# StefanSko/mcmc-db

Measured on AMD Instinct MI355X. Metric: validated param-draws/sec, higher is better.
Workload: dtype f64; 1 GPU; single posteriordb-shaped model, 4x10000x100 synthetic draws per GPU (BASELINE config 1; AR(1) chains, ties and a shifted chain; SURVEY 8(d) C1); layout=pcn, statistics=mean,std,q5,q50,q95,split_rhat,ess_bulk,ess_tail

## Files before the change

mcmc-db_amd/csrc/mcr_device.hpp:

```cpp
#pragma once
#include <hip/hip_runtime.h>
#include <stdint.h>

namespace mcr {

using i64 = long long;
using u32 = unsigned int;
using u64 = unsigned long long;

constexpr int kWave = 64;

template <int CTRL>
__device__ __forceinline__ double dpp_f64(double v)
{
    const int lo = __builtin_amdgcn_mov_dpp(__double2loint(v), CTRL, 0xf, 0xf, true);
    const int hi = __builtin_amdgcn_mov_dpp(__double2hiint(v), CTRL, 0xf, 0xf, true);
    return __hiloint2double(hi, lo);
}
__device__ __forceinline__ double readlane_f64(double v, int lane)
{
    return __hiloint2double(__builtin_amdgcn_readlane(__double2hiint(v), lane),
                            __builtin_amdgcn_readlane(__double2loint(v), lane));
}
constexpr int kDppXor1 = 0xB1, kDppXor2 = 0x4E, kDppRor4 = 0x124, kDppRor8 = 0x128;

__device__ __forceinline__ double row_sum(double v)
{
    v += dpp_f64<kDppXor1>(v); v += dpp_f64<kDppXor2>(v); v += dpp_f64<kDppRor4>(v); v += dpp_f64<kDppRor8>(v);
    return v;
}
template <int CTRL>
__device__ __forceinline__ u32 dpp_u32(u32 v) { return (u32)__builtin_amdgcn_mov_dpp((int)v, CTRL, 0xf, 0xf, true); }
__device__ __forceinline__ u32 row_min_u32(u32 v)
{
    v = min(v, dpp_u32<kDppXor1>(v)); v = min(v, dpp_u32<kDppXor2>(v));
    v = min(v, dpp_u32<kDppRor4>(v)); v = min(v, dpp_u32<kDppRor8>(v));
    return v;
}
__device__ __forceinline__ u32 row_max_u32(u32 v)
{
    v = max(v, dpp_u32<kDppXor1>(v)); v = max(v, dpp_u32<kDppXor2>(v));
    v = max(v, dpp_u32<kDppRor4>(v)); v = max(v, dpp_u32<kDppRor8>(v));
    return v;
}
__device__ __forceinline__ double wave_sum(double v)
{
    v = row_sum(v);
    return (readlane_f64(v, 0) + readlane_f64(v, 16)) + (readlane_f64(v, 32) + readlane_f64(v, 48));
}
template <int CTRL, int ROW_MASK>
__device__ __forceinline__ double dpp_f64_or_zero(double v)
{
    const int lo = __builtin_amdgcn_update_dpp(0, __double2loint(v), CTRL, ROW_MASK, 0xf, false);
    const int hi = __builtin_amdgcn_update_dpp(0, __double2hiint(v), CTRL, ROW_MASK, 0xf, false);
    return __hiloint2double(hi, lo);
}
__device__ __forceinline__ double wave_excl_scan(double v, double& total)
{
    double incl = v;
    incl += dpp_f64_or_zero<0x111, 0xf>(incl);
    incl += dpp_f64_or_zero<0x112, 0xf>(incl);
    incl += dpp_f64_or_zero<0x114, 0xf>(incl);
    incl += dpp_f64_or_zero<0x118, 0xf>(incl);
    incl += dpp_f64_or_zero<0x142, 0xa>(incl);
    incl += dpp_f64_or_zero<0x143, 0xc>(incl);
    total = readlane_f64(incl, 63);
    return incl - v;
}

__device__ __forceinline__ int row_lane(int v, int j)
{
#define MCR_RL(J) case J: return __builtin_amdgcn_update_dpp(0, v, 0x150 + J, 0xf, 0xf, false);
    switch (j & 15) {
        MCR_RL(0) MCR_RL(1) MCR_RL(2) MCR_RL(3) MCR_RL(4) MCR_RL(5) MCR_RL(6) MCR_RL(7)
        MCR_RL(8) MCR_RL(9) MCR_RL(10) MCR_RL(11) MCR_RL(12) MCR_RL(13) MCR_RL(14)
        default: return __builtin_amdgcn_update_dpp(0, v, 0x15F, 0xf, 0xf, false);
    }
#undef MCR_RL
}

template <int CTRL, int ROW_MASK, int OLD>
__device__ __forceinline__ int dpp_i32_or(int v) { return __builtin_amdgcn_update_dpp(OLD, v, CTRL, ROW_MASK, 0xf, false); }

__device__ __forceinline__ u32 wave_excl_scan_u32(u32 v, u32& total)
{
    int incl = (int)v;
    incl += dpp_i32_or<0x111, 0xf, 0>(incl); incl += dpp_i32_or<0x112, 0xf, 0>(incl);
    incl += dpp_i32_or<0x114, 0xf, 0>(incl); incl += dpp_i32_or<0x118, 0xf, 0>(incl);
    incl += dpp_i32_or<0x142, 0xa, 0>(incl);
    incl += dpp_i32_or<0x143, 0xc, 0>(incl);
    total = (u32)__builtin_amdgcn_readlane(incl, 63);
    return (u32)incl - v;
}

__device__ __forceinline__ int wave_prefix_max(int v, int& excl)
{
    v = max(v, dpp_i32_or<0x111, 0xf, -1>(v)); v = max(v, dpp_i32_or<0x112, 0xf, -1>(v));
    v = max(v, dpp_i32_or<0x114, 0xf, -1>(v)); v = max(v, dpp_i32_or<0x118, 0xf, -1>(v));
    v = max(v, dpp_i32_or<0x142, 0xa, -1>(v)); v = max(v, dpp_i32_or<0x143, 0xc, -1>(v));
    excl = dpp_i32_or<0x138, 0xf, -1>(v);
    return v;
}
__device__ __forceinline__ int wave_suffix_min(int v, int& excl)
{
    constexpr int kMax = 0x7fffffff;
    v = min(v, dpp_i32_or<0x101, 0xf, kMax>(v)); v = min(v, dpp_i32_or<0x102, 0xf, kMax>(v));
    v = min(v, dpp_i32_or<0x104, 0xf, kMax>(v)); v = min(v, dpp_i32_or<0x108, 0xf, kMax>(v));
    const int r1 = __builtin_amdgcn_readlane(v, 16), r2 = __builtin_amdgcn_readlane(v, 32), r3 = __builtin_amdgcn_readlane(v, 48);
    const int row = (threadIdx.x & 63) >> 4;
    const int m23 = min(r2, r3), m123 = min(r1, m23);
    const int above = (row == 0) ? m123 : ((row == 1) ? m23 : ((row == 2) ? r3 : kMax));
    v = min(v, above);
    excl = dpp_i32_or<0x130, 0xf, kMax>(v);
    return v;
}

template <int NT>
__device__ __forceinline__ double block_sum(double v, double* red)
{
    v = wave_sum(v);
    __syncthreads();
    if ((threadIdx.x & 63) == 0) red[threadIdx.x >> 6] = v;
    __syncthreads();
    double r = 0.0;
#pragma unroll
    for (int w = 0; w < NT / kWave; ++w) r += red[w];
    return r;
// ... 143 lines not shown
```

mcmc-db_amd/csrc/mcr_diag.hpp:

```cpp
#pragma once
#include "mcr_device.hpp"

namespace mcr {

constexpr int kSeg = 2048;
#ifndef MCR_LAG1
#define MCR_LAG1 64
#endif
constexpr int kLag1 = MCR_LAG1;
constexpr int kSegRec = kLag1 + 12;
constexpr int kMoreBlocks = 3;
constexpr int kLag2 = kLag1 + 64 * kMoreBlocks;
constexpr int kLongGroup = 256;
constexpr int kLongSlots = 2;
enum SegField { SG_S = kLag1, SG_S0, SG_Q0, SG_S1, SG_Q1, SG_MIN, SG_MAX, SG_MIN0, SG_MAX0, SG_MIN1, SG_MAX1 };

__device__ __forceinline__ i64 pos8(i64 j) { return j + ((j >> 3) << 1); }

__device__ __forceinline__ double zdec(const double* __restrict__ ztab, u32 code, i64 M)
{
    const u32 cmax = (u32)(2 * M - 1);
    return ztab[code < cmax ? code : cmax];
}

// ... 39 lines not shown
    }
    __syncthreads();
    if (ph == 0) {
#pragma unroll
        for (int li = 0; li < LPL; ++li) wred[w * 64 + g * LPL + li] = acc[li];
    }
    __syncthreads();
    if (tid < LPL * LG) {
        double t = 0.0;
#pragma unroll
        for (int ww = 0; ww < NW; ++ww) t += wred[ww * 64 + tid];
        tot[tid] = t;
    }
    __syncthreads();
}

template <int NT, int LG = 8>
__device__ __forceinline__ void seg_reduce_rows(double (&acc)[8], double* tot, double* scr)
{
    constexpr int NW = NT / kWave;
    static_assert(LG == 8 || LG == 4, "8 or 4 lag groups of 8 lags");
    const int tid = threadIdx.x, lane = tid & 63, w = tid >> 6;
    const int g = lane & (LG - 1), row = lane >> 4;
#pragma unroll
    for (int li = 0; li < 8; ++li) {
        if (LG == 4) acc[li] += dpp_f64<kDppRor4>(acc[li]);
        acc[li] += dpp_f64<kDppRor8>(acc[li]);
    }
    __syncthreads();
    if ((lane & 15) < LG) {
#pragma unroll
        for (int li = 0; li < 8; ++li) scr[(w * 4 + row) * 64 + g * 8 + li] = acc[li];
    }
    __syncthreads();
    if (tid < LG * 8) {
        double t = 0.0;
#pragma unroll
        for (int r = 0; r < NW * 4; ++r) t += scr[r * 64 + tid];
        tot[tid] = t;
    }
    __syncthreads();
}

template <int NT, int SEG, bool FIRST>
__global__ __launch_bounds__(NT) void k_acov_seg(const u32* __restrict__ zb, const u32* __restrict__ zt,
                                                 const double* __restrict__ ztab, i64 M,
                                                 const i64* __restrict__ off, int C, i64 n, i64 nh, int nseg,
                                                 const unsigned* __restrict__ more, double* __restrict__ rec, int kind_sel)
{
    constexpr int NW = NT / kWave;
    static_assert(SEG % 128 == 0, "spans of the widest tile are 128 draws");
    static_assert(kLag1 == 64 || kLag1 == 32, "tier 1 is one or half a lag block");
    constexpr int WIN = FIRST ? SEG + 80 : SEG + 64 * kMoreBlocks + 80;
    constexpr int LX = WIN / 8 * 10;
    constexpr int NLD = (WIN + NT - 1) / NT;
    static_assert(LX >= NW * 4 * 64, "the reduction scratch aliases the staged window");
    __shared__ __attribute__((aligned(16))) double sx[LX];
    __shared__ __attribute__((aligned(16))) double scr2[FIRST ? 8 : NW * 4 * 64];
    __shared__ double tot[64];
    __shared__ double wred[NW * 4 * 8];

    const int tid = threadIdx.x;
    const int seg = blockIdx.x, c = blockIdx.y;
    const i64 pk = (kind_sel < 0) ? (i64)blockIdx.z : 2 * (i64)blockIdx.z + kind_sel, p = pk >> 1;
    const int kind = (int)(pk & 1);
    if (!FIRST && more[pk] == 0u) return;
    const u32* zc = (kind ? zt : zb) + p * M + off[c];
    const i64 nc = off[c + 1] - off[c], hc = nc / 2;
    const i64 hspan = (hc > 0) ? hc + nh : 0;
    const i64 nload = (n > hspan) ? n : hspan;
    const i64 s0 = (i64)seg * SEG;
    const int seglen = (int)((n - s0 < 0) ? 0 : ((n - s0 < (i64)SEG) ? n - s0 : (i64)SEG));

    if (FIRST) {
        auto rel = [&](i64 x) -> int { const i64 d = x - s0; return (int)(d < 0 ? 0 : (d > WIN ? WIN : d)); };
        const int r_load = rel(nload);
        const int r_n = rel(n);
        const int own = (r_load < SEG) ? r_load : SEG;
        const int own_n = (own < r_n) ? own : r_n;
        auto clip = [&](int x) -> int { return x < own ? x : own; };
        const int a0 = (hc > 0) ? clip(rel(0)) : 0, a1 = (hc > 0) ? clip(rel(nh)) : 0;
        const int b0 = (hc > 0) ? clip(rel(hc)) : 0, b1 = (hc > 0) ? clip(rel(hc + nh)) : 0;
        double S = 0.0, S0 = 0.0, Q0 = 0.0, S1 = 0.0, Q1 = 0.0;
        u32 cmin = 0xFFFFFFFFu, cmax = 0u;
        u32 c0min = 0xFFFFFFFFu, c0max = 0u, c1min = 0xFFFFFFFFu, c1max = 0u;
        double v[NLD];
        u32 cd[NLD];
#pragma unroll
        for (int u = 0; u < NLD; ++u) {
            const int j = u * NT + tid;
            cd[u] = (j < r_load) ? zc[s0 + j] : 0u;
            v[u] = (j < r_load) ? zdec(ztab, cd[u], M) : 0.0;
        }
        const int jw0 = __builtin_amdgcn_readfirstlane(tid & ~63);
#define MCR_IN_WINDOW(lo, hi, BODY)                                                        \
        if (jw >= (lo) && jw + 64 <= (hi)) { BODY }                                        \
        else if (jw + 64 > (lo) && jw < (hi)) { if (j >= (lo) && j < (hi)) { BODY } }
#pragma unroll
        for (int u = 0; u < NLD; ++u) {
            const int jw = u * NT + jw0, j = u * NT + tid;
            const double x = v[u];
            MCR_IN_WINDOW(0, own_n, S += x; cmin = min(cmin, cd[u]); cmax = max(cmax, cd[u]);)
            MCR_IN_WINDOW(a0, a1, S0 += x; Q0 = fma(x, x, Q0); c0min = min(c0min, cd[u]); c0max = max(c0max, cd[u]);)
            MCR_IN_WINDOW(b0, b1, S1 += x; Q1 = fma(x, x, Q1); c1min = min(c1min, cd[u]); c1max = max(c1max, cd[u]);)
            if (j < WIN) sx[pos8(j)] = (j < r_n) ? x : 0.0;
        }
#undef MCR_IN_WINDOW
        S = row_sum(S); S0 = row_sum(S0); Q0 = row_sum(Q0); S1 = row_sum(S1); Q1 = row_sum(Q1);
        cmin = row_min_u32(cmin); cmax = row_max_u32(cmax);
        c0min = row_min_u32(c0min); c0max = row_max_u32(c0max); c1min = row_min_u32(c1min); c1max = row_max_u32(c1max);
        static_assert(NW * 4 * 4 <= 64, "the four half-window fields of every DPP row fit `tot`");
        if ((tid & 15) == 0) {
            double* q = wred + (tid >> 4) * 8;
            q[0] = S; q[1] = S0; q[2] = Q0; q[3] = S1; q[4] = Q1; q[5] = (double)cmin; q[6] = (double)cmax;
            double* q2 = tot + (tid >> 4) * 4;
            q2[0] = (double)c0min; q2[1] = (double)c0max; q2[2] = (double)c1min; q2[3] = (double)c1max;
        }
        __syncthreads();
        double* r = rec + ((pk * C + c) * (i64)nseg + seg) * kSegRec;
        if (tid < 11) {
            const double* src = (tid < 7) ? wred + tid : tot + (tid - 7);
            const int stride = (tid < 7) ? 8 : 4;
            double t = src[0];
            for (int w = 1; w < NW * 4; ++w) {
                const double x = src[w * stride];
                t = (tid < 5) ? t + x : (((tid & 1) == 1) ? fmin(t, x) : fmax(t, x));
            }
            r[SG_S + tid] = t;
        }
        double acc[8];
#pragma unroll
        for (int i = 0; i < 8; ++i) acc[i] = 0.0;
        seg_accumulate<NT, kLag1 / 8, 8>(sx, sx, seglen, acc);
        seg_reduce_rows<NT, kLag1 / 8>(acc, tot, sx);
        if (tid < kLag1) r[tid] = tot[tid];
    } else {
        double* r = rec + ((pk * C + c) * (i64)nseg + seg) * (64 * kMoreBlocks);
        if (seglen == 0) {
            for (int j = tid; j < 64 * kMoreBlocks; j += NT) r[j] = 0.0;
            return;
        }
        double v[NLD];
#pragma unroll
        for (int u = 0; u < NLD; ++u) {
            const int j = u * NT + tid;
            v[u] = (j < WIN && s0 + j < n) ? zdec(ztab, zc[s0 + j], M) : 0.0;
        }
#pragma unroll
        for (int u = 0; u < NLD; ++u) {
            const int j = u * NT + tid;
            if (j < WIN) sx[pos8(j)] = v[u];
        }
        __syncthreads();
        for (int blk = 0; blk < kMoreBlocks; ++blk) {
            const int lb = kLag1 + 64 * blk;
            double acc[8];
#pragma unroll
            for (int i = 0; i < 8; ++i) acc[i] = 0.0;
            seg_accumulate<NT, 8, 8>(sx, sx + 10 * (lb >> 3), seglen, acc);
            seg_reduce_rows<NT>(acc, tot, scr2);
            if (tid < 64) r[blk * 64 + tid] = tot[tid];
        }
    }
}

constexpr int kT3StageGroups = 8, kT3Stages = 9;
constexpr unsigned kT3Prev = 0x80000000u;
__host__ __device__ constexpr int t3_stage_first(int st, int groups)
{
    return groups <= kT3StageGroups ? (st == 0 ? 0 : groups) : (st == 0 ? 0 : (st == 1 ? 2 : kT3StageGroups * (st - 1)));
}

constexpr int kChState = 6;
constexpr int kPairState = 4;

constexpr double kRhoBand = 1e-10;
constexpr int kGuardMax = 64;

__device__ __forceinline__ int guard_budget(i64 n)
{
    const i64 b = (n <= 32768) ? (i64)kGuardMax : ((i64)kGuardMax * 32768) / n;
    return (int)(b < 4 ? 4 : b);
}

constexpr int kGuardChains12 = 4, kGuardChunk12 = 128;
constexpr int kGuardChains = 8, kGuardChunk = 256;
template <int CH, int CK>
struct GuardLds {
    double gA[CH][CK], gB[CH][CK];
    double gcov[CH], gmean[CH];
    double gsum;
};

template <int CH, int CK>
__device__ __noinline__ double ref_cov_sum(const u32* __restrict__ z, const double* __restrict__ ztab, i64 M,
                                           const i64* __restrict__ off, int C, i64 n, i64 lag,
                                           double* __restrict__ chst, GuardLds<CH, CK>& G)
{
#pragma clang fp contract(off)
    const int tid = threadIdx.x, NT = (int)blockDim.x;
    __syncthreads();
    if (tid == 0) G.gsum = 0.0;
    const i64 len = n - lag;
    for (int c0 = 0; c0 < C; c0 += CH) {
        const int nc = (C - c0 < CH) ? C - c0 : CH;
        __syncthreads();
        if (tid < nc) G.gmean[tid] = chst[(c0 + tid) * kChState + 5];
        __syncthreads();
        bool need = false;
        for (int c = 0; c < nc; ++c) need = need || (G.gmean[c] != G.gmean[c]);
        if (need) {
// ... 636 lines not shown
```

mcmc-db_amd/csrc/mcr_kernels.hpp:

```cpp
#pragma once
#include "mcr_device.hpp"
#include "mcr_sortnet.h"

namespace mcr {

enum ResField {
    R_MEAN = 0, R_STD, R_MEDIAN, R_RHAT, R_RHAT_BULK, R_RHAT_TAIL, R_ESS_BULK, R_ESS_TAIL,
    R_LAG_BULK, R_LAG_TAIL, R_BAD, R_Q0
};

#ifndef MCR_WCOMB
#define MCR_WCOMB 1
#endif
constexpr bool kWriteCombine = MCR_WCOMB != 0;

struct QArgs {
    int nq;
    i64 lo[32];
    double g[32];
};

__device__ __forceinline__ bool xcd_map(i64 P, int nb, i64& p, int& blk)
{
    const i64 L = blockIdx.x;
    const i64 xcd = L & 7, j = L >> 3;
    p = (j / nb) * 8 + xcd;
    blk = (int)(j % nb);
    return p < P;
}

__global__ __launch_bounds__(256) void k_ztable(double* __restrict__ ztab, i64 M)
{
    const i64 n2 = (i64)blockIdx.x * 256 + threadIdx.x;
    if (n2 >= 2 * M) return;
    const double r = (double)(n2 + 1) / 2.0;
    ztab[n2] = (n2 >= 1) ? inv_cdf((r - 0.5) / (double)M) : 0.0;
}

__global__ __launch_bounds__(256) void k_decode_codes(const u32* __restrict__ code, const double* __restrict__ ztab,
                                                      i64 n, double* __restrict__ z, double* __restrict__ rank)
{
    const i64 i = (i64)blockIdx.x * 256 + threadIdx.x;
    if (i >= n) return;
    u32 c = code[i];
    if ((i64)c > 2 * n - 1) c = (u32)(2 * n - 1);
    if (z) z[i] = ztab[c];
    if (rank) rank[i] = (double)((i64)c + 1) / 2.0;
}

template <typename T>
__global__ __launch_bounds__(256) void k_ingest_rows(const T* __restrict__ src, double* __restrict__ X,
                                                     i64 C, i64 N, i64 sc, i64 sn, i64 sp, i64 p0)
{
    const i64 nb = (N + 255) / 256;
    const i64 c = blockIdx.x / nb, t = (blockIdx.x % nb) * 256 + threadIdx.x;
    const i64 p = blockIdx.y;
    if (t < N) X[p * (C * N) + c * N + t] = (double)src[c * sc + t * sn + (p0 + p) * sp];
}

template <typename T>
__global__ __launch_bounds__(256) void k_ingest_transpose(const T* __restrict__ src,
                                                          double* __restrict__ X, i64 C, i64 N, i64 P,
                                                          i64 sc, i64 sn, i64 sp, i64 p0)
{
    __shared__ double tile[64][65];
    const i64 nb = (N + 63) / 64;
    const i64 c = blockIdx.x / nb, t0 = (blockIdx.x % nb) * 64;
    const i64 pl0 = (i64)blockIdx.y * 64;
    const int tx = threadIdx.x & 63, ty = threadIdx.x >> 6;
    for (int r = ty; r < 64; r += 4) {
        const i64 t = t0 + r, p = pl0 + tx;
        tile[r][tx] = (t < N && p < P) ? (double)src[c * sc + t * sn + (p0 + p) * sp] : 0.0;
    }
    __syncthreads();
    for (int q = ty; q < 64; q += 4) {
        const i64 t = t0 + tx, p = pl0 + q;
        if (t < N && p < P) X[p * (C * N) + c * N + t] = tile[tx][q];
    }
}

constexpr int kMomRec = 5;

__device__ __forceinline__ void store_slice_moments(double* o, double K, double s1, double s2, double bad, double n)
// ... 172 lines not shown
            const double o_s = dpp_f64<CTRL>(k[r]);
            const u32 oi_s = dpp_u32<CTRL>(ix[r]);
            exchange(k[s], ix[s], o_s, oi_s);
        }
        exchange(k[r], ix[r], o_r, oi_r);
    }
}

__device__ __forceinline__ void lane_bitonic_merge16(double (&k)[16], u32 (&ix)[16])
{
#define MCR_CE(a, b)                                                        \
    {                                                                       \
        const bool sw = k[b] < k[a];                                        \
        const double lo = sw ? k[b] : k[a], hi = sw ? k[a] : k[b];          \
        const u32 ilo = sw ? ix[b] : ix[a], ihi = sw ? ix[a] : ix[b];       \
        k[a] = lo; k[b] = hi; ix[a] = ilo; ix[b] = ihi;                     \
    }
    MCR_BITONIC16(MCR_CE)
#undef MCR_CE
}

__device__ __forceinline__ void lane_merge_levels_16_to_64(double (&k)[16], u32 (&ix)[16])
{
    constexpr unsigned long long kEvenLanes = 0x5555555555555555ull, kLowPairs = 0x3333333333333333ull;
    lane_pair_stage<0xB1, true, kEvenLanes>(k, ix);
    lane_bitonic_merge16(k, ix);
    lane_pair_stage<0x1B, true, kLowPairs>(k, ix);
    lane_pair_stage<0xB1, false, kEvenLanes>(k, ix);
    lane_bitonic_merge16(k, ix);
#if MCR_TILE_DPP_LEVELS >= 3
    constexpr unsigned long long kLowQuads = 0x0F0F0F0F0F0F0F0Full;
    lane_pair_stage<0x141, true, kLowQuads>(k, ix);
    lane_pair_stage<0x4E, false, kLowPairs>(k, ix);
    lane_pair_stage<0xB1, false, kEvenLanes>(k, ix);
    lane_bitonic_merge16(k, ix);
#endif
}

template <int VT>
__device__ __forceinline__ void serial_merge(const double* skey, int a0, int na, int b0, int nb, int ai,
                                             int bi, int nout, double (&k)[VT], int (&src)[VT])
{
    int pa = a0 + ai, pb = b0 + bi;
    const int ea = a0 + na, eb = b0 + nb;
    double ak = skey[pos16(pa)], bk = skey[pos16(pb)];
#pragma unroll
    for (int i = 0; i < VT; ++i) {
        if (i < nout) {
            const bool takeA = (pb >= eb) | ((pa < ea) & !(bk < ak));
            k[i] = takeA ? ak : bk;
            src[i] = takeA ? pa : pb;
            pa += takeA ? 1 : 0;
            pb += takeA ? 0 : 1;
            const int pn = takeA ? pa : pb;
            const double nv = skey[pos16(pn)];
            ak = takeA ? nv : ak;
            bk = takeA ? bk : nv;
        } else {
            src[i] = 0;
        }
    }
}

template <typename IdxT> constexpr size_t sort_lds_bytes(int T) { return (size_t)T * (8 + sizeof(IdxT)); }

template <int NT, int VT, typename IdxT, typename XT>
__global__ __launch_bounds__(NT) void k_tile_sort(const XT* __restrict__ X, i64 M,
                                                  double* __restrict__ keys, IdxT* __restrict__ idx,
                                                  double* __restrict__ part, int ntiles,
                                                  double* __restrict__ samp)
{
    constexpr int T = NT * VT;
    extern __shared__ __attribute__((aligned(16))) char smem[];
    double* skey = reinterpret_cast<double*>(smem);
    IdxT* sidx = reinterpret_cast<IdxT*>(skey + T);
    double* red = skey;

    const int tid = threadIdx.x, tile = blockIdx.x;
    const i64 p = blockIdx.y;
    const i64 base = (i64)tile * T;
    const int count = (int)((M - base < (i64)T) ? M - base : (i64)T);
    const XT* src = X + p * M + base;

    double bad = 0.0;
#pragma unroll
    for (int i = 0; i < VT; ++i) {
        const int e = i * NT + tid;
        double v = INFINITY;
        if (e < count) {
            v = (double)src[e];
            bad += isfinite(v) ? 0.0 : 1.0;
        }
        skey[pos16(e)] = v;
    }
    __syncthreads();

    double k[VT];
    u32 ix[VT];
#pragma unroll
    for (int i = 0; i < VT; ++i) {
        const int e = tid * VT + i;
        k[i] = skey[pos16(e)];
        ix[i] = (e < count) ? (u32)(base + e) : 0xFFFFFFFFu;
    }
    thread_sort<VT>(k, ix);
    constexpr bool kLaneLevels = MCR_TILE_DPP_LEVELS >= 2 && VT == 16;
    if constexpr (kLaneLevels) lane_merge_levels_16_to_64(k, ix);
    __syncthreads();
#pragma unroll
    for (int i = 0; i < VT; ++i) {
        const int e = tid * VT + i;
        skey[pos16(e)] = k[i];
        sidx[posi(e)] = (IdxT)ix[i];
    }
    __syncthreads();

    for (int coop = kLaneLevels ? (MCR_TILE_DPP_LEVELS >= 3 ? 16 : 8) : 2; coop <= NT; coop <<= 1) {
        const int first = tid & ~(coop - 1);
        const int run = VT * (coop >> 1);
        const int a0 = first * VT, b0 = a0 + run;
        const int diag = VT * (tid - first);
        auto A = [&](int i) { return skey[pos16(a0 + i)]; };
        auto B = [&](int j) { return skey[pos16(b0 + j)]; };
        const int ai = merge_path32(A, run, B, run, diag);
        int srcs[VT];
        serial_merge<VT>(skey, a0, run, b0, run, ai, diag - ai, VT, k, srcs);
#pragma unroll
        for (int i = 0; i < VT; ++i) ix[i] = sidx[posi(srcs[i])];
        __syncthreads();
#pragma unroll
        for (int i = 0; i < VT; ++i) {
            const int e = tid * VT + i;
            skey[pos16(e)] = k[i];
            sidx[posi(e)] = (IdxT)ix[i];
        }
        __syncthreads();
    }

    for (int e = tid; e < count; e += NT) {
        keys[p * M + base + e] = skey[pos16(e)];
        idx[p * M + base + e] = sidx[posi(e)];
    }
    if (samp != nullptr && tid < T / 64) {
        const int e = 64 * tid + 63;
        samp[(p * ntiles + tile) * (T / 64) + tid] = (e < count) ? skey[pos16(e)] : INFINITY;
    }
    __syncthreads();
    double s1 = 0.0;
#pragma unroll
    for (int i = 0; i < VT; ++i) s1 += (tid * VT + i < count) ? k[i] : 0.0;
    s1 = block_sum<NT>(s1, red);
    const double mt = s1 / (double)count;
    double s2 = 0.0, e1 = 0.0;
#pragma unroll
    for (int i = 0; i < VT; ++i) { const double d = (tid * VT + i < count) ? k[i] - mt : 0.0; s2 = fma(d, d, s2); e1 += d; }
    block_sum3<NT>(s2, e1, bad, red);
    if (tid == 0) store_slice_moments(part + (p * ntiles + tile) * kMomRec, mt, e1, s2, bad, (double)count);
}

template <int NT, int VT>
__device__ __forceinline__ void scatter_codes_by_line(u32* __restrict__ zrow, i64 M, int total, const u32 (&hcode)[VT],
                                                      const u32 (&hpos)[VT], u32* cnt_code, unsigned short* spos, u32* swt)
{
    constexpr int kMaxLines = 2048, PER = kMaxLines / NT > 0 ? kMaxLines / NT : 1;
    static_assert(NT * PER >= kMaxLines, "every line counter has an owner in the scan");
    const int tid = threadIdx.x;
    const int nlines = (int)((M + 31) >> 5);
    u32* scnt = cnt_code;
    u32* scode = cnt_code + 2112;
    __syncthreads();
    for (int i = tid; i <= nlines; i += NT) scnt[i] = 0u;
    __syncthreads();
    u32 rk[VT];
#pragma unroll
    for (int i = 0; i < VT; ++i) rk[i] = (tid * VT + i < total) ? atomicAdd(&scnt[hpos[i] >> 5], 1u) : 0u;
    __syncthreads();
    {
        u32 c[PER], tsum = 0;
#pragma unroll
        for (int j = 0; j < PER; ++j) { const int q = tid * PER + j; c[j] = (q < nlines) ? scnt[q] : 0u; tsum += c[j]; }
        u32 wtot;
        const u32 wex = wave_excl_scan_u32(tsum, wtot);
        if ((tid & 63) == 0) swt[tid >> 6] = wtot;
        __syncthreads();
        u32 base = wex;
        for (int w = 0; w < (tid >> 6); ++w) base += swt[w];
#pragma unroll
        for (int j = 0; j < PER; ++j) { const int q = tid * PER + j; if (q < nlines) scnt[q] = base; base += c[j]; }
    }
    __syncthreads();
#pragma unroll
    for (int i = 0; i < VT; ++i) {
        if (tid * VT + i < total) {
            const u32 slot = min(scnt[hpos[i] >> 5] + rk[i], (u32)(NT * VT - 1));
            scode[slot] = hcode[i];
            spos[slot] = (unsigned short)hpos[i];
        }
    }
    __syncthreads();
    for (int e = tid; e < total; e += NT) zrow[spos[e]] = scode[e];
}

template <int NT, int VT, class KF>
__device__ __forceinline__ void block_tie_runs(KF key_at, int total, int* wsh, int (&rs)[VT], int (&re)[VT])
{
    constexpr int NW = NT / kWave;
    const int tid = threadIdx.x, lane = tid & 63, w = tid >> 6;
    const int base = tid * VT;
    bool h[VT];
    auto prev = key_at((base > 0 && base - 1 < total) ? base - 1 : 0);
    int cur = -1, first = 0x7fffffff;
#pragma unroll
    for (int i = 0; i < VT; ++i) {
        const int g = base + i;
        const auto kv = key_at(g < total ? g : 0);
        h[i] = (g == 0) || (g >= total) || (prev != kv);
        if (h[i]) { cur = g; if (first == 0x7fffffff) first = g; }
        rs[i] = cur;
        prev = kv;
    }
    int exL, exR;
    const int incl = wave_prefix_max(cur, exL);
    const int rinc = wave_suffix_min(first, exR);
    __syncthreads();
    if (lane == 63) wsh[w] = incl;
    if (lane == 0) wsh[NW + w] = rinc;
    __syncthreads();
    int carryL = -1, carryR = total;
#pragma unroll
    for (int ww = 0; ww < NW; ++ww) {
        if (ww < w) carryL = max(carryL, wsh[ww]);
        if (ww > w) carryR = min(carryR, wsh[NW + ww]);
    }
    carryL = max(carryL, exL);
    carryR = min(carryR, exR);
    if (carryR > total) carryR = total;
    int nxt = carryR;
#pragma unroll
// ... 643 lines not shown
```

mcmc-db_amd/csrc/mcr_sort32.hpp:

```cpp
#pragma once
#include "mcr_kernels.hpp"

namespace mcr {

__device__ __forceinline__ u32 rec_key(u64 r) { return (u32)(r >> 32); }
__device__ __forceinline__ u32 rec_pos(u64 r) { return (u32)r; }

template <int VT>
__device__ __forceinline__ void thread_sort_rec(u64 (&r)[VT])
{
    static_assert(VT == 16 || VT == 8, "sorting networks exist for 16 and 8 items per lane");
#define MCR_CE(a, b)                                         \
    {                                                        \
        const bool sw = r[b] < r[a];                         \
        const u64 lo = sw ? r[b] : r[a], hi = sw ? r[a] : r[b]; \
        r[a] = lo; r[b] = hi;                                \
    }
    if constexpr (VT == 16) { MCR_NET16(MCR_CE) } else { MCR_NET8(MCR_CE) }
#undef MCR_CE
}

template <int CTRL>
__device__ __forceinline__ u64 dpp_u64(u64 v)
{
// ... 12 lines not shown
        own = select_by_mask(own, o, (lt & MIN_LANES) | (gt & ~MIN_LANES));
    };
#pragma unroll
    for (int i = 0; i < (MIRROR ? 8 : 16); ++i) {
        const int s = MIRROR ? 15 - i : i;
        const u64 o_i = dpp_u64<CTRL>(r[s]);
        if (MIRROR) {
            const u64 o_s = dpp_u64<CTRL>(r[i]);
            exchange(r[s], o_s);
        }
        exchange(r[i], o_i);
    }
}

__device__ __forceinline__ void lane_bitonic_merge16_rec(u64 (&r)[16])
{
#define MCR_CE(a, b)                                         \
    {                                                        \
        const bool sw = r[b] < r[a];                         \
        const u64 lo = sw ? r[b] : r[a], hi = sw ? r[a] : r[b]; \
        r[a] = lo; r[b] = hi;                                \
    }
    MCR_BITONIC16(MCR_CE)
#undef MCR_CE
}

__device__ __forceinline__ void lane_merge_levels_rec(u64 (&r)[16])
{
    constexpr unsigned long long kEvenLanes = 0x5555555555555555ull, kLowPairs = 0x3333333333333333ull,
                                 kLowQuads = 0x0F0F0F0F0F0F0F0Full;
    lane_pair_stage_rec<0xB1, true, kEvenLanes>(r);
    lane_bitonic_merge16_rec(r);
    lane_pair_stage_rec<0x1B, true, kLowPairs>(r);
    lane_pair_stage_rec<0xB1, false, kEvenLanes>(r);
    lane_bitonic_merge16_rec(r);
    lane_pair_stage_rec<0x141, true, kLowQuads>(r);
    lane_pair_stage_rec<0x4E, false, kLowPairs>(r);
    lane_pair_stage_rec<0xB1, false, kEvenLanes>(r);
    lane_bitonic_merge16_rec(r);
}

template <int VT, int LIM = 0>
__device__ __forceinline__ void serial_merge_rec(const u64* srec, int a0, int na, int b0, int nb, int ai, int bi,
                                                 int nout, u64 (&out)[VT])
{
    int pa = a0 + ai, pb = b0 + bi;
    const int ea = a0 + na, eb = b0 + nb;
    auto slot = [](int e) { return pos16(LIM > 0 ? min(e, LIM) : e); };
    u64 ar = srec[slot(pa)], br = srec[slot(pb)];
#pragma unroll
    for (int i = 0; i < VT; ++i) {
        if (i < nout) {
            const bool takeA = (pb >= eb) | ((pa < ea) & !(br < ar));
            out[i] = takeA ? ar : br;
            pa += takeA ? 1 : 0;
            pb += takeA ? 0 : 1;
            const int pn = takeA ? pa : pb;
            const u64 nv = srec[slot(pn)];
            ar = takeA ? nv : ar;
            br = takeA ? br : nv;
        } else {
            out[i] = kRecPad;
        }
    }
}

constexpr size_t rec_lds_bytes(int T) { return (size_t)(T + 2) * 8; }

template <int NT, int VT>
__global__ __launch_bounds__(NT) void k_tile_sort32(const float* __restrict__ X, i64 M, u64* __restrict__ recs,
                                                    double* __restrict__ part, int ntiles, double* __restrict__ samp)
{
    constexpr int T = NT * VT;
    extern __shared__ __attribute__((aligned(16))) char smem[];
    u64* srec = reinterpret_cast<u64*>(smem);
    double* red = reinterpret_cast<double*>(smem);

    const int tid = threadIdx.x, tile = blockIdx.x;
    const i64 p = blockIdx.y;
    const i64 base = (i64)tile * T;
    const int count = (int)((M - base < (i64)T) ? M - base : (i64)T);
    const float* src = X + p * M + base;

    double bad = 0.0;
#pragma unroll
    for (int i = 0; i < VT; ++i) {
        const int e = i * NT + tid;
        u64 r = kRecPad;
        if (e < count) {
            const float v = src[e];
            bad += isfinite(v) ? 0.0 : 1.0;
            r = ((u64)f32_key(v) << 32) | (u64)(u32)(base + e);
        }
        srec[pos16(e)] = r;
    }
    __syncthreads();
    u64 r[VT];
#pragma unroll
    for (int i = 0; i < VT; ++i) r[i] = srec[pos16(tid * VT + i)];
    thread_sort_rec<VT>(r);
    constexpr bool kLaneLevels = MCR_TILE_DPP_LEVELS >= 3 && VT == 16;
    if constexpr (kLaneLevels) lane_merge_levels_rec(r);
    __syncthreads();
#pragma unroll
    for (int i = 0; i < VT; ++i) srec[pos16(tid * VT + i)] = r[i];
    __syncthreads();

    for (int coop = kLaneLevels ? 16 : 2; coop <= NT; coop <<= 1) {
        const int first = tid & ~(coop - 1);
        const int run = VT * (coop >> 1);
        const int a0 = first * VT, b0 = a0 + run;
        const int diag = VT * (tid - first);
        auto A = [&](int i) { return srec[pos16(a0 + i)]; };
        auto B = [&](int j) { return srec[pos16(b0 + j)]; };
        const int ai = merge_path32(A, run, B, run, diag);
        serial_merge_rec<VT, T - 1>(srec, a0, run, b0, run, ai, diag - ai, VT, r);
        __syncthreads();
#pragma unroll
        for (int i = 0; i < VT; ++i) srec[pos16(tid * VT + i)] = r[i];
        __syncthreads();
    }
    for (int e = tid; e < count; e += NT) recs[p * M + base + e] = srec[pos16(e)];
    if (samp != nullptr && tid < T / 64) {
        const int e = 64 * tid + 63;
        samp[(p * ntiles + tile) * (T / 64) + tid] = (e < count) ? key_value(rec_key(srec[pos16(e)])) : INFINITY;
    }
    __syncthreads();
    double s1 = 0.0;
#pragma unroll
    for (int i = 0; i < VT; ++i) s1 += (tid * VT + i < count) ? key_value(rec_key(r[i])) : 0.0;
    s1 = block_sum<NT>(s1, red);
    const double mt = s1 / (double)count;
    double s2 = 0.0, e1 = 0.0;
#pragma unroll
    for (int i = 0; i < VT; ++i) { const double d = (tid * VT + i < count) ? key_value(rec_key(r[i])) - mt : 0.0; s2 = fma(d, d, s2); e1 += d; }
    block_sum3<NT>(s2, e1, bad, red);
    if (tid == 0) store_slice_moments(part + (p * ntiles + tile) * kMomRec, mt, e1, s2, bad, (double)count);
}

template <int NT, int VT>
__global__ __launch_bounds__(NT) void k_merge32(const u64* __restrict__ rin, u64* __restrict__ rout, i64 M, i64 R)
{
    constexpr int OB = NT * VT;
    extern __shared__ __attribute__((aligned(16))) char smem[];
    u64* srec = reinterpret_cast<u64*>(smem);
    __shared__ i64 sh[2];
    const int tid = threadIdx.x;
    const i64 p = blockIdx.y;
    const i64 o0 = (i64)blockIdx.x * OB;
    if (o0 >= M) return;
    const u64* rp = rin + p * M;
    const i64 pb = (o0 / (2 * R)) * (2 * R);
    const i64 abase = pb, na = (M - pb < R) ? M - pb : R;
    const i64 bbase = pb + na, nb = (M - bbase < R) ? M - bbase : R;
    const i64 d0 = o0 - pb, tot = na + nb;
    const i64 d1 = (d0 + OB < tot) ? d0 + OB : tot;
    auto GA = [&](i64 i) { return rp[abase + i]; };
    auto GB = [&](i64 j) { return rp[bbase + j]; };
    if (tid < 64) { const i64 r0 = merge_path_wave(GA, na, GB, nb, d0); if (tid == 0) sh[0] = r0; }
    else if (tid < 128) { const i64 r1 = merge_path_wave(GA, na, GB, nb, d1); if (tid == 64) sh[1] = r1; }
    __syncthreads();
    const i64 ai0 = sh[0], ai1 = sh[1], bi0 = d0 - ai0;
    const int ca = (int)(ai1 - ai0), cb = (int)((d1 - ai1) - bi0);
    const int total = ca + cb;
    {
        u64 gr[VT];
#pragma unroll
        for (int j = 0; j < VT; ++j) {
            const int e = j * NT + tid;
            const i64 g = (e < ca) ? abase + ai0 + e : bbase + bi0 + (e - ca);
            gr[j] = rp[(e < total) ? g : 0];
        }
#pragma unroll
        for (int j = 0; j < VT; ++j) {
            const int e = j * NT + tid;
            if (e < total) srec[pos16(e)] = gr[j];
        }
    }
    __syncthreads();
    const int diag = (tid * VT < total) ? tid * VT : total;
    const int nout = (total - diag < VT) ? total - diag : VT;
    auto A = [&](int i) { return srec[pos16(i)]; };
    auto B = [&](int j) { return srec[pos16(ca + j)]; };
    const int ai = merge_path32(A, ca, B, cb, diag);
    u64 r[VT];
    serial_merge_rec<VT>(srec, 0, ca, ca, cb, ai, diag - ai, nout, r);
    __syncthreads();
#pragma unroll
    for (int i = 0; i < VT; ++i)
        if (i < nout) srec[pos16(diag + i)] = r[i];
    __syncthreads();
    for (int e = tid; e < total; e += NT) rout[p * M + o0 + e] = srec[pos16(e)];
}

template <int NT, int VT>
__global__ __launch_bounds__(NT) void k_bucket_merge32(const u64* __restrict__ rin, u64* __restrict__ rout, i64 M,
                                                       int k, int B, const u32* __restrict__ cut,
                                                       const u32* __restrict__ boff, u32* __restrict__ z, i64 P, i64 R)
{
    constexpr int T = NT * VT;
    static_assert(T == 4096, "the partition bound of k_splitters assumes 4096-slot buckets");
    extern __shared__ __attribute__((aligned(16))) char smem[];
    u64* srec = reinterpret_cast<u64*>(smem);
    int* sst = reinterpret_cast<int*>(srec + T + 2);
    int* spl = sst + 40;
    int* sps = spl + 40;
    i64* sedge = reinterpret_cast<i64*>(sps + 40);

    const int tid = threadIdx.x;
    i64 p;
    int b;
    if (!xcd_map(P, B, p, b)) return;
    const u64* rp = rin + p * M;
    const u32* c0 = cut + (p * (B + 1) + b) * k;
    const u32* c1 = c0 + k;
    if (tid == 0) {
        int acc = 0;
        for (int t = 0; t < k; ++t) {
// ... 122 lines not shown
```

Baseline: 24.29 billion param-draws/s.

## Replace rank min/max with ballot constancy flags and load tile-sort keys directly

The first diagnostics pass no longer tracks per-window min/max of rank codes through DPP reductions. It compares each code against a reference code with a wave ballot and stores a single 'not constant' flag, writing min=0 and max=flag in the segment record. The tile-sort kernels (f64 and f32 record paths) now load keys straight into registers in striped order instead of staging through LDS with barriers. They also specialize full tiles at compile time, which removes bounds checks in load, write-out and moment loops. Downstream code must interpret min/max only as a constancy test. The striped register load also changes which elements each thread sorts, and correctness relies on the later merge stages.

After: 25.24 billion param-draws/s, median of 6. 1.04x the previous value.

```diff
diff --git a/mcmc-db_amd/csrc/mcr_device.hpp b/mcmc-db_amd/csrc/mcr_device.hpp
--- a/mcmc-db_amd/csrc/mcr_device.hpp
+++ b/mcmc-db_amd/csrc/mcr_device.hpp
@@ -31,18 +31,6 @@
 }
 template <int CTRL>
 __device__ __forceinline__ u32 dpp_u32(u32 v) { return (u32)__builtin_amdgcn_mov_dpp((int)v, CTRL, 0xf, 0xf, true); }
-__device__ __forceinline__ u32 row_min_u32(u32 v)
-{
-    v = min(v, dpp_u32<kDppXor1>(v)); v = min(v, dpp_u32<kDppXor2>(v));
-    v = min(v, dpp_u32<kDppRor4>(v)); v = min(v, dpp_u32<kDppRor8>(v));
-    return v;
-}
-__device__ __forceinline__ u32 row_max_u32(u32 v)
-{
-    v = max(v, dpp_u32<kDppXor1>(v)); v = max(v, dpp_u32<kDppXor2>(v));
-    v = max(v, dpp_u32<kDppRor4>(v)); v = max(v, dpp_u32<kDppRor8>(v));
-    return v;
-}
 __device__ __forceinline__ double wave_sum(double v)
 {
     v = row_sum(v);
diff --git a/mcmc-db_amd/csrc/mcr_diag.hpp b/mcmc-db_amd/csrc/mcr_diag.hpp
--- a/mcmc-db_amd/csrc/mcr_diag.hpp
+++ b/mcmc-db_amd/csrc/mcr_diag.hpp
@@ -145,8 +145,8 @@
         const int a0 = (hc > 0) ? clip(rel(0)) : 0, a1 = (hc > 0) ? clip(rel(nh)) : 0;
         const int b0 = (hc > 0) ? clip(rel(hc)) : 0, b1 = (hc > 0) ? clip(rel(hc + nh)) : 0;
         double S = 0.0, S0 = 0.0, Q0 = 0.0, S1 = 0.0, Q1 = 0.0;
-        u32 cmin = 0xFFFFFFFFu, cmax = 0u;
-        u32 c0min = 0xFFFFFFFFu, c0max = 0u, c1min = 0xFFFFFFFFu, c1max = 0u;
+        const u32 ref0 = (nc > 0) ? zc[0] : 0u, ref1 = (hc > 0) ? zc[hc] : 0u;
+        unsigned long long dif = 0ull, dif0 = 0ull, dif1 = 0ull;
         double v[NLD];
         u32 cd[NLD];
 #pragma unroll
@@ -156,40 +156,40 @@
             v[u] = (j < r_load) ? zdec(ztab, cd[u], M) : 0.0;
         }
         const int jw0 = __builtin_amdgcn_readfirstlane(tid & ~63);
-#define MCR_IN_WINDOW(lo, hi, BODY)                                                        \
-        if (jw >= (lo) && jw + 64 <= (hi)) { BODY }                                        \
-        else if (jw + 64 > (lo) && jw < (hi)) { if (j >= (lo) && j < (hi)) { BODY } }
+#define MCR_IN_WINDOW(lo, hi, DIF, REF, BODY)                                              \
+        if (jw >= (lo) && jw + 64 <= (hi)) { BODY DIF |= __builtin_amdgcn_ballot_w64(cd[u] != (REF)); } \
+        else if (jw + 64 > (lo) && jw < (hi)) {                                            \
+            const bool in = j >= (lo) && j < (hi);                                         \
+            DIF |= __builtin_amdgcn_ballot_w64(in && cd[u] != (REF));                      \
+            if (in) { BODY }                                                               \
+        }
 #pragma unroll
         for (int u = 0; u < NLD; ++u) {
             const int jw = u * NT + jw0, j = u * NT + tid;
             const double x = v[u];
-            MCR_IN_WINDOW(0, own_n, S += x; cmin = min(cmin, cd[u]); cmax = max(cmax, cd[u]);)
-            MCR_IN_WINDOW(a0, a1, S0 += x; Q0 = fma(x, x, Q0); c0min = min(c0min, cd[u]); c0max = max(c0max, cd[u]);)
-            MCR_IN_WINDOW(b0, b1, S1 += x; Q1 = fma(x, x, Q1); c1min = min(c1min, cd[u]); c1max = max(c1max, cd[u]);)
+            MCR_IN_WINDOW(0, own_n, dif, ref0, S += x;)
+            MCR_IN_WINDOW(a0, a1, dif0, ref0, S0 += x; Q0 = fma(x, x, Q0);)
+            MCR_IN_WINDOW(b0, b1, dif1, ref1, S1 += x; Q1 = fma(x, x, Q1);)
             if (j < WIN) sx[pos8(j)] = (j < r_n) ? x : 0.0;
         }
 #undef MCR_IN_WINDOW
         S = row_sum(S); S0 = row_sum(S0); Q0 = row_sum(Q0); S1 = row_sum(S1); Q1 = row_sum(Q1);
-        cmin = row_min_u32(cmin); cmax = row_max_u32(cmax);
-        c0min = row_min_u32(c0min); c0max = row_max_u32(c0max); c1min = row_min_u32(c1min); c1max = row_max_u32(c1max);
-        static_assert(NW * 4 * 4 <= 64, "the four half-window fields of every DPP row fit `tot`");
         if ((tid & 15) == 0) {
             double* q = wred + (tid >> 4) * 8;
-            q[0] = S; q[1] = S0; q[2] = Q0; q[3] = S1; q[4] = Q1; q[5] = (double)cmin; q[6] = (double)cmax;
-            double* q2 = tot + (tid >> 4) * 4;
-            q2[0] = (double)c0min; q2[1] = (double)c0max; q2[2] = (double)c1min; q2[3] = (double)c1max;
+            q[0] = S; q[1] = S0; q[2] = Q0; q[3] = S1; q[4] = Q1;
+            q[5] = dif ? 1.0 : 0.0; q[6] = dif0 ? 1.0 : 0.0; q[7] = dif1 ? 1.0 : 0.0;
         }
         __syncthreads();
         double* r = rec + ((pk * C + c) * (i64)nseg + seg) * kSegRec;
-        if (tid < 11) {
-            const double* src = (tid < 7) ? wred + tid : tot + (tid - 7);
-            const int stride = (tid < 7) ? 8 : 4;
+        if (tid < 8) {
+            const double* src = wred + tid;
             double t = src[0];
             for (int w = 1; w < NW * 4; ++w) {
-                const double x = src[w * stride];
-                t = (tid < 5) ? t + x : (((tid & 1) == 1) ? fmin(t, x) : fmax(t, x));
+                const double x = src[w * 8];
+                t = (tid < 5) ? t + x : fmax(t, x);
             }
-            r[SG_S + tid] = t;
+            if (tid < 5) r[SG_S + tid] = t;
+            else { r[SG_MIN + 2 * (tid - 5)] = 0.0; r[SG_MAX + 2 * (tid - 5)] = t; }
         }
         double acc[8];
 #pragma unroll
diff --git a/mcmc-db_amd/csrc/mcr_kernels.hpp b/mcmc-db_amd/csrc/mcr_kernels.hpp
--- a/mcmc-db_amd/csrc/mcr_kernels.hpp
+++ b/mcmc-db_amd/csrc/mcr_kernels.hpp
@@ -1,4 +1,5 @@
 #pragma once
+#include <type_traits>
 #include "mcr_device.hpp"
 #include "mcr_sortnet.h"
 
@@ -337,31 +338,26 @@
     const int count = (int)((M - base < (i64)T) ? M - base : (i64)T);
     const XT* src = X + p * M + base;
 
-    double bad = 0.0;
-#pragma unroll
-    for (int i = 0; i < VT; ++i) {
-        const int e = i * NT + tid;
-        double v = INFINITY;
-        if (e < count) {
-            v = (double)src[e];
-            bad += isfinite(v) ? 0.0 : 1.0;
-        }
-        skey[pos16(e)] = v;
-    }
-    __syncthreads();
-
+    const bool full = count == T;
     double k[VT];
     u32 ix[VT];
-#pragma unroll
-    for (int i = 0; i < VT; ++i) {
-        const int e = tid * VT + i;
-        k[i] = skey[pos16(e)];
-        ix[i] = (e < count) ? (u32)(base + e) : 0xFFFFFFFFu;
-    }
+    double bad = 0.0;
+    auto load = [&](auto full_c) {
+        constexpr bool FULL = decltype(full_c)::value;
+#pragma unroll
+        for (int i = 0; i < VT; ++i) {
+            const int e = i * NT + tid;
+            const bool live = FULL || e < count;
+            const double v = (double)src[FULL ? e : min(e, count - 1)];
+            k[i] = live ? v : INFINITY;
+            ix[i] = live ? (u32)(base + e) : 0xFFFFFFFFu;
+            bad += (live && !isfinite(v)) ? 1.0 : 0.0;
+        }
+    };
+    if (full) load(std::true_type{}); else load(std::false_type{});
     thread_sort<VT>(k, ix);
     constexpr bool kLaneLevels = MCR_TILE_DPP_LEVELS >= 2 && VT == 16;
     if constexpr (kLaneLevels) lane_merge_levels_16_to_64(k, ix);
-    __syncthreads();
 #pragma unroll
     for (int i = 0; i < VT; ++i) {
         const int e = tid * VT + i;
@@ -392,23 +388,32 @@
         __syncthreads();
     }
 
-    for (int e = tid; e < count; e += NT) {
-        keys[p * M + base + e] = skey[pos16(e)];
-        idx[p * M + base + e] = sidx[posi(e)];
-    }
+    auto write_out = [&](auto full_c) {
+        constexpr bool FULL = decltype(full_c)::value;
+#pragma nounroll
+        for (int e = tid; e < (FULL ? T : count); e += NT) {
+            keys[p * M + base + e] = skey[pos16(e)];
+            idx[p * M + base + e] = sidx[posi(e)];
+        }
+    };
+    if (full) write_out(std::true_type{}); else write_out(std::false_type{});
     if (samp != nullptr && tid < T / 64) {
         const int e = 64 * tid + 63;
         samp[(p * ntiles + tile) * (T / 64) + tid] = (e < count) ? skey[pos16(e)] : INFINITY;
     }
     __syncthreads();
-    double s1 = 0.0;
-#pragma unroll
-    for (int i = 0; i < VT; ++i) s1 += (tid * VT + i < count) ? k[i] : 0.0;
-    s1 = block_sum<NT>(s1, red);
-    const double mt = s1 / (double)count;
-    double s2 = 0.0, e1 = 0.0;
-#pragma unroll
-    for (int i = 0; i < VT; ++i) { const double d = (tid * VT + i < count) ? k[i] - mt : 0.0; s2 = fma(d, d, s2); e1 += d; }
+    double s1 = 0.0, s2 = 0.0, e1 = 0.0, mt = 0.0;
+    auto moments = [&](auto full_c) {
+        constexpr bool FULL = decltype(full_c)::value;
+        const int nlive = count - tid * VT;
+#pragma unroll
+        for (int i = 0; i < VT; ++i) s1 += (FULL || i < nlive) ? k[i] : 0.0;
+        s1 = block_sum<NT>(s1, red);
+        mt = s1 / (double)count;
+#pragma unroll
+        for (int i = 0; i < VT; ++i) { const double d = (FULL || i < nlive) ? k[i] - mt : 0.0; s2 = fma(d, d, s2); e1 += d; }
+    };
+    if (full) moments(std::true_type{}); else moments(std::false_type{});
     block_sum3<NT>(s2, e1, bad, red);
     if (tid == 0) store_slice_moments(part + (p * ntiles + tile) * kMomRec, mt, e1, s2, bad, (double)count);
 }
diff --git a/mcmc-db_amd/csrc/mcr_sort32.hpp b/mcmc-db_amd/csrc/mcr_sort32.hpp
--- a/mcmc-db_amd/csrc/mcr_sort32.hpp
+++ b/mcmc-db_amd/csrc/mcr_sort32.hpp
@@ -118,26 +118,24 @@
     const int count = (int)((M - base < (i64)T) ? M - base : (i64)T);
     const float* src = X + p * M + base;
 
+    const bool full = count == T;
+    u64 r[VT];
     double bad = 0.0;
-#pragma unroll
-    for (int i = 0; i < VT; ++i) {
-        const int e = i * NT + tid;
-        u64 r = kRecPad;
-        if (e < count) {
-            const float v = src[e];
-            bad += isfinite(v) ? 0.0 : 1.0;
-            r = ((u64)f32_key(v) << 32) | (u64)(u32)(base + e);
-        }
-        srec[pos16(e)] = r;
-    }
-    __syncthreads();
-    u64 r[VT];
-#pragma unroll
-    for (int i = 0; i < VT; ++i) r[i] = srec[pos16(tid * VT + i)];
+    auto load = [&](auto full_c) {
+        constexpr bool FULL = decltype(full_c)::value;
+#pragma unroll
+        for (int i = 0; i < VT; ++i) {
+            const int e = i * NT + tid;
+            const bool live = FULL || e < count;
+            const float v = src[FULL ? e : min(e, count - 1)];
+            bad += (live && !isfinite(v)) ? 1.0 : 0.0;
+            r[i] = live ? (((u64)f32_key(v) << 32) | (u64)(u32)(base + e)) : kRecPad;
+        }
+    };
+    if (full) load(std::true_type{}); else load(std::false_type{});
     thread_sort_rec<VT>(r);
     constexpr bool kLaneLevels = MCR_TILE_DPP_LEVELS >= 3 && VT == 16;
     if constexpr (kLaneLevels) lane_merge_levels_rec(r);
-    __syncthreads();
 #pragma unroll
     for (int i = 0; i < VT; ++i) srec[pos16(tid * VT + i)] = r[i];
     __syncthreads();
@@ -156,20 +154,29 @@
         for (int i = 0; i < VT; ++i) srec[pos16(tid * VT + i)] = r[i];
         __syncthreads();
     }
-    for (int e = tid; e < count; e += NT) recs[p * M + base + e] = srec[pos16(e)];
+    auto write_out = [&](auto full_c) {
+        constexpr bool FULL = decltype(full_c)::value;
+#pragma nounroll
+        for (int e = tid; e < (FULL ? T : count); e += NT) recs[p * M + base + e] = srec[pos16(e)];
+    };
+    if (full) write_out(std::true_type{}); else write_out(std::false_type{});
     if (samp != nullptr && tid < T / 64) {
         const int e = 64 * tid + 63;
         samp[(p * ntiles + tile) * (T / 64) + tid] = (e < count) ? key_value(rec_key(srec[pos16(e)])) : INFINITY;
     }
     __syncthreads();
-    double s1 = 0.0;
-#pragma unroll
-    for (int i = 0; i < VT; ++i) s1 += (tid * VT + i < count) ? key_value(rec_key(r[i])) : 0.0;
-    s1 = block_sum<NT>(s1, red);
-    const double mt = s1 / (double)count;
-    double s2 = 0.0, e1 = 0.0;
-#pragma unroll
-    for (int i = 0; i < VT; ++i) { const double d = (tid * VT + i < count) ? key_value(rec_key(r[i])) - mt : 0.0; s2 = fma(d, d, s2); e1 += d; }
+    double s1 = 0.0, s2 = 0.0, e1 = 0.0, mt = 0.0;
+    auto moments = [&](auto full_c) {
+        constexpr bool FULL = decltype(full_c)::value;
+        const int nlive = count - tid * VT;
+#pragma unroll
+        for (int i = 0; i < VT; ++i) s1 += (FULL || i < nlive) ? key_value(rec_key(r[i])) : 0.0;
+        s1 = block_sum<NT>(s1, red);
+        mt = s1 / (double)count;
+#pragma unroll
+        for (int i = 0; i < VT; ++i) { const double d = (FULL || i < nlive) ? key_value(rec_key(r[i])) - mt : 0.0; s2 = fma(d, d, s2); e1 += d; }
+    };
+    if (full) moments(std::true_type{}); else moments(std::false_type{});
     block_sum3<NT>(s2, e1, bad, red);
     if (tid == 0) store_slice_moments(part + (p * ntiles + tile) * kMomRec, mt, e1, s2, bad, (double)count);
 }
```
